# zipnn/zipnn

Measured on AMD Instinct MI355X. Metric: bf16 decompress GB/s (uncompressed bytes / s; compress GB/s beside it), higher is better.
Workload: dtype u8; 1 GPU; 4 GiB synthetic bf16 N(0,0.02) tensor per GPU, 256 KiB chunks, byte-split + huff0 (BASELINE.json configs[1]); chunks_per_gpu=16384, parallelism=chunk-sharded x1, no collectives

## Files before the change

zipnn_amd/csrc/zn_decode_chain.hpp:

```cpp
#pragma once

#include "zn_common.hpp"

#ifndef ZN_F_TLMAX
#define ZN_F_TLMAX 11u
#endif
#ifndef ZN_IN_IDX
#define ZN_IN_IDX(i) (i)
#endif
#if !defined(ZN_SIMT_EMULATOR)
#define ZN_STEP_FENCE() __builtin_amdgcn_sched_barrier(0)
#else
#define ZN_STEP_FENCE() do { } while (0)
#endif

#define ZN_E_META(cnt, nb, efields) ((nb) | ((cnt) << 8) | (efields))
#define ZN_M_NB(m) ((m) & 15u)
#define ZN_M_CNT(m) (((m) >> 8) & 7u)

__device__ __forceinline__ uint32_t zn_wave_excl_scan(uint32_t v, uint32_t lane, uint32_t* total) {
  int x = (int)v;
  x += __builtin_amdgcn_update_dpp(0, x, 0x111, 0xF, 0xF, false);
  x += __builtin_amdgcn_update_dpp(0, x, 0x112, 0xF, 0xF, false);
  x += __builtin_amdgcn_update_dpp(0, x, 0x114, 0xF, 0xF, false);
  x += __builtin_amdgcn_update_dpp(0, x, 0x118, 0xF, 0xF, false);
  x += __builtin_amdgcn_update_dpp(0, x, 0x142, 0xA, 0xF, false);
  x += __builtin_amdgcn_update_dpp(0, x, 0x143, 0xC, 0xF, false);
  *total = (uint32_t)__builtin_amdgcn_readlane(x, 63);
  (void)lane;
  return (uint32_t)x - v;
}

__device__ __forceinline__ uint64_t zn_window(const uint32_t* in, int32_t q) {
  q = q < 32 ? 32 : q;
  const int32_t j = q >> 5; const uint32_t sh = 31u - (uint32_t)(q & 31);
  const uint32_t d1 = in[ZN_IN_IDX(j)], d0 = in[ZN_IN_IDX(j - 1)];
  return (((uint64_t)d1 << 32) | d0) << sh;
}

__device__ __forceinline__ uint2 zn_trim_group(uint2 e, int32_t rem) {
  const uint32_t meta = e.y;
  const uint32_t have = ZN_M_CNT(meta);
  const uint32_t k0 = (uint32_t)(rem > 0) + (uint32_t)((int32_t)((meta >> 16) & 15u) < rem) + (uint32_t)((int32_t)((meta >> 20) & 15u) < rem) +
                      (uint32_t)((int32_t)((meta >> 24) & 15u) < rem);
  const uint32_t k = k0 < have ? k0 : have;
  const uint32_t F = ((meta >> 16) & 0xFFFu) | (ZN_M_NB(meta) << 12);
  const uint32_t nbk = k ? ((F >> (4u * k - 4u)) & 15u) : 0u;
  uint2 r;
  r.x = e.x & (k >= 4u ? 0xFFFFFFFFu : ~(0xFFFFFFFFu << (8u * k)));
  r.y = nbk | (k << 8);
  return r;
}

__device__ __forceinline__ uint2 zn_trim_group_dense(uint2 e, int32_t rem) {
  const uint32_t meta = e.y;
  const uint32_t nb = ZN_M_NB(meta), e1 = (meta >> 16) & 15u;
  const bool t0 = rem > 0, t1 = (int32_t)e1 < rem && ZN_M_CNT(meta) >= 2u;
  uint2 r;
  r.x = t1 ? e.x : (t0 ? (e.x & 0xFFu) : 0u);
  r.y = t1 ? (nb | (2u << 8)) : (t0 ? (e1 | (1u << 8)) : 0u);
  return r;
}

struct ZnChain {
  int32_t pos, stop;
  uint32_t n;
  uint32_t wpos;
};
template <int MODE>
__device__ __forceinline__ void zn_chain_apply(ZnChain& c, uint2 e, uint32_t* stage) {
  if (MODE == 2) {
    const uint64_t sp = (uint64_t)e.x << ((c.wpos & 3u) << 3);
    uint32_t* d = (uint32_t*)((uint8_t*)stage + (c.wpos & ~3u));
    if ((uint32_t)sp) atomicOr(d, (uint32_t)sp);
    if ((uint32_t)(sp >> 32)) atomicOr(d + 1, (uint32_t)(sp >> 32));
    c.wpos += ZN_M_CNT(e.y);
  }
  if (MODE == 1) c.n += ZN_M_CNT(e.y);
  c.pos -= (int32_t)ZN_M_NB(e.y);
}
template <int MODE, bool DENSE = false>
__device__ __forceinline__ void zn_fused_run(const uint2* lut, const uint32_t* in, int32_t base_bit, uint32_t TL, ZnChain& c, uint32_t* stage, int U = 0) {
  const uint32_t sh = 32u - TL;
  const int32_t mb = c.stop + (int32_t)TL - 1;
  for (int u = 0; u + 3 <= U; u += 3) {
    uint64_t w = zn_window(in, c.pos - 1 - base_bit);
    for (int s = 0; s < 3; s++) {
      const uint2 e = lut[(uint32_t)(w >> 32) >> sh];
      w <<= (e.y & 63u);
      zn_chain_apply<MODE>(c, e, stage);
    }
  }
  while (__any(c.pos > mb)) {
    uint64_t w = zn_window(in, c.pos - 1 - base_bit);
    for (int s = 0; s < 3; s++) {
      uint2 e = lut[(uint32_t)(w >> 32) >> sh];
      if (!(c.pos > mb)) { e.x = 0; e.y = 0; }
      w <<= (e.y & 63u);
      zn_chain_apply<MODE>(c, e, stage);
    }
  }
  while (__any(c.pos > c.stop)) {
    const uint64_t w = zn_window(in, c.pos - 1 - base_bit);
    uint2 e = lut[(uint32_t)(w >> 32) >> sh];
    if (!DENSE && !(c.pos > c.stop)) { e.x = 0; e.y = 0; }
    zn_chain_apply<MODE>(c, DENSE ? zn_trim_group_dense(e, c.pos - c.stop) : zn_trim_group(e, c.pos - c.stop), stage);
  }
}

#if defined(ZN_SIMT_EMULATOR)
__device__ __forceinline__ uint32_t zn_alignbyte(uint32_t hi, uint32_t lo, uint32_t sh) { return (uint32_t)(((((uint64_t)hi) << 32) | lo) >> (8u * (sh & 3u))); }
#else
__device__ __forceinline__ uint32_t zn_alignbyte(uint32_t hi, uint32_t lo, uint32_t sh) { return __builtin_amdgcn_alignbyte(hi, lo, sh); }
#endif

#define ZN_REC_LIST(X) X(0) X(1) X(2) X(3) X(4) X(5) X(6) X(7) X(8) X(9) X(10) X(11) X(12) X(13) X(14) X(15) X(16) X(17) X(18) X(19) \
                       X(20) X(21) X(22) X(23) X(24) X(25) X(26) X(27)
#define ZN_REC_MAX 28
struct ZnRec {
#define X(i) uint32_t s##i;
  ZN_REC_LIST(X)
#undef X
  uint32_t c0, c1, c2, c3, c4, c5, c6;
};
template <int I> __device__ __forceinline__ uint32_t& zn_rec_s(ZnRec& r) {
#define X(i) if constexpr (I == i) return r.s##i; else
  ZN_REC_LIST(X) return r.s0;
#undef X
}
template <int G> __device__ __forceinline__ uint32_t& zn_rec_c(ZnRec& r) {
  if constexpr (G == 0) return r.c0; else if constexpr (G == 1) return r.c1; else if constexpr (G == 2) return r.c2;
  else if constexpr (G == 3) return r.c3; else if constexpr (G == 4) return r.c4; else if constexpr (G == 5) return r.c5; else return r.c6;
}
template <int I, bool DENSE = false> __device__ __forceinline__ void zn_rec_put(ZnRec& r, uint32_t syms, uint32_t meta) {
  if constexpr (DENSE) { uint32_t& sr = zn_rec_s<I / 2>(r); if constexpr (I % 2 == 0) sr = syms; else sr = __builtin_amdgcn_perm(syms, sr, 0x05040100u); }
  else zn_rec_s<I>(r) = syms;
  constexpr uint32_t sel = (I % 4 == 0) ? 0x03020105u : (I % 4 == 1) ? 0x03020500u : (I % 4 == 2) ? 0x03050100u : 0x05020100u;
  uint32_t& c = zn_rec_c<I / 4>(r);
  c = __builtin_amdgcn_perm(meta, c, sel);
}
template <int I> __device__ __forceinline__ uint32_t zn_rec_cnt(ZnRec& r) { return (zn_rec_c<I / 4>(r) >> (8 * (I % 4))) & 7u; }
template <int I, bool DENSE> __device__ __forceinline__ uint32_t zn_rec_sym(ZnRec& r) {
  if constexpr (DENSE) return (I % 2 == 0) ? (zn_rec_s<I / 2>(r) & 0xFFFFu) : (zn_rec_s<I / 2>(r) >> 16);
  else return zn_rec_s<I>(r);
}
template <int N> struct ZnIdx { static constexpr int v = N; };
template <int I, int N, typename F> __device__ __forceinline__ void zn_static_for(F&& f) {
  if constexpr (I < N) { f(ZnIdx<I>{}); zn_static_for<I + 1, N>(f); }
}

template <int TF, int TB, int U, bool DENSE = false>
__device__ __forceinline__ bool zn_pass1(const uint2* lut, const uint32_t* in, int32_t base_bit, uint32_t TL, int32_t pos0, int32_t stop,
                                         bool own, ZnRec& rec, uint32_t& acc_out, int& nfull, int& nbnd) {
  static_assert(TF + TB <= ZN_REC_MAX, "more record slots than ZnRec has");
  const uint32_t sh = 32u - TL;
  const int32_t R = own ? pos0 - stop : -1000;
  const int32_t lim_full = R - (int32_t)TL + 1;
  const int32_t qb = pos0 - 1 - base_bit;
  uint64_t w = 0;
  uint32_t acc = 0;
  int t_end = TF; bool live = true;
  zn_static_for<0, TF>([&](auto I) {
    constexpr int t = decltype(I)::v;
    constexpr bool checked = t >= U;
    if (live) {
      bool act = true;
      if (checked) {
        act = (int32_t)(acc & 0xFFu) < lim_full;
        if (!__any(act)) { t_end = t; live = false; }
      }
      if (live) {
        if (t % 3 == 0) w = zn_window(in, qb - (int32_t)(acc & 0xFFu));
        uint2 e = lut[(uint32_t)(w >> 32) >> sh];
        if (checked && !act) { e.x = 0; e.y = 0; }
        w <<= (e.y & 63u);
        acc += e.y;
        zn_rec_put<t, DENSE>(rec, e.x, e.y);
        ZN_STEP_FENCE();
      }
    }
  });
  if (live && __any((int32_t)(acc & 0xFFu) < lim_full)) return false;
  int b_end = TB; live = true;
  zn_static_for<0, TB>([&](auto I) {
    constexpr int b = decltype(I)::v;
    if (live) {
      const int32_t rem = R - (int32_t)(acc & 0xFFu);
      if (!__any(rem > 0)) { b_end = b; live = false; }
      if (live) {
        w = zn_window(in, qb - (int32_t)(acc & 0xFFu));
        uint2 e = lut[(uint32_t)(w >> 32) >> sh];
        if (!DENSE && !(rem > 0)) { e.x = 0; e.y = 0; }
        e = DENSE ? zn_trim_group_dense(e, rem) : zn_trim_group(e, rem);
        acc += e.y;
        zn_rec_put<TF + b, DENSE>(rec, e.x, e.y);
        ZN_STEP_FENCE();
      }
    }
  });
  nfull = __builtin_amdgcn_readfirstlane(t_end); nbnd = __builtin_amdgcn_readfirstlane(b_end);
  acc_out = acc;
  return true;
}

template <int TF, int TB, bool DENSE = false, uint32_t AMASK = ~3u, typename HOOK>
__device__ __forceinline__ void zn_pass2(uint32_t* stage, uint32_t wpos, ZnRec& rec, int nfull, int nbnd, HOOK&& hook) {
  uint32_t wm1 = wpos - 1u;
  auto put = [&](uint32_t cnt, uint32_t sv) {
    const uint32_t g = ~wm1;
    uint32_t* d = (uint32_t*)((uint8_t*)stage + (int32_t)(wm1 & AMASK));
    const uint32_t lo = zn_alignbyte(sv, 0u, g), hi = zn_alignbyte(0u, sv, g);
    if (lo) atomicOr(d, lo);
    if (hi) atomicOr(d + 1, hi);
    wm1 += cnt;
    ZN_STEP_FENCE();
  };
  if constexpr (DENSE) {
    zn_static_for<0, (TF + TB + 1) / 2>([&](auto R_) {
      constexpr int r = decltype(R_)::v, a = 2 * r, b = 2 * r + 1;
      const bool va = a < TF ? a < nfull : (a - TF) < nbnd;
      const bool vb = b < TF + TB && (b < TF ? b < nfull : (b - TF) < nbnd);
      if (va || vb) {
        uint32_t ca = 0, cb = 0;
        if (va) ca = zn_rec_cnt<a>(rec);
        if constexpr (b < TF + TB) { if (vb) cb = zn_rec_cnt<b>(rec); }
        const uint32_t sr = zn_rec_s<r>(rec);
        const uint32_t sel = (ca >= 2u) ? 0x03020100u : (ca == 1u) ? 0x0c030200u : 0x0c0c0302u;
        put(ca + cb, __builtin_amdgcn_perm(sr, sr, sel));
        if (va) hook(ZnIdx<a>{});
        if constexpr (b < TF + TB) { if (vb) hook(ZnIdx<b>{}); }
      }
    });
  } else {
    zn_static_for<0, TF>([&](auto I) { constexpr int t = decltype(I)::v; if (t < nfull) { put(zn_rec_cnt<t>(rec), zn_rec_sym<t, DENSE>(rec)); hook(I); } });
    zn_static_for<0, TB>([&](auto I) { constexpr int b = decltype(I)::v; if (b < nbnd) { put(zn_rec_cnt<TF + b>(rec), zn_rec_sym<TF + b, DENSE>(rec)); hook(ZnIdx<TF + b>{}); } });
  }
}
```

zipnn_amd/csrc/zn_decode_fused.hip:

```cpp
#include "zn_internal.hpp"
#include <atomic>
#include "zn_huf_wave.hpp"
#include "zn_decode_common.hpp"
#include "zn_decode_rest.hpp"

#define ZN_F_THREADS 256
#define ZN_F_RING_BYTES 4096u
#define ZN_F_WAVES_PER_SIMD 4
#define ZN_F_RING_DW (ZN_F_RING_BYTES / 4u)
#define ZN_F_DMAX 6
#define ZN_F_DCAP 4
#define ZN_F_DOM_MAX 154
#define ZN_F_DCONST 4
#define ZN_F_DCONST2 6
#define ZN_F_DENSE_LMIN 4
#define ZN_F_IN_DW (64 * ZN_F_DMAX + 4)
#define ZN_F_TF(D) ((D) * 4 + 1)
#define ZN_F_TLMAX 11u
#define ZN_L16(i) ((i) + (((i) >> 6) << 1))
#define ZN_F_PRIO_SYNC 1
#define ZN_F_PRIO_COUNT 2
#define ZN_F_PRIO_WRITE 3
#if !defined(ZN_SIMT_EMULATOR)
#define ZN_PRIO(v) __builtin_amdgcn_s_setprio(v)
#else
#define ZN_PRIO(v) do { } while (0)
#endif
#if !defined(ZN_SIMT_EMULATOR)
#define ZN_OPAQUE32(x) asm volatile("" : "+v"(x))
#define ZN_KEEP32(x) asm volatile("" :: "v"(x))
__device__ __forceinline__ uint32_t zn_bfi_(uint32_t mask, uint32_t a, uint32_t b) {
  uint32_t d; asm("v_bfi_b32 %0, %1, %2, %3" : "=v"(d) : "s"(mask), "v"(a), "v"(b)); return d;
}
#define ZN_BFI(mask, a, b) zn_bfi_((mask), (a), (b))
#define ZN_NO_IFCVT asm volatile("")
#define ZN_ASM_MARK(txt) asm volatile("; " txt)
#else
#define ZN_NO_IFCVT ((void)0)
#define ZN_ASM_MARK(txt) ((void)0)
#define ZN_OPAQUE32(x) ((void)0)
#define ZN_KEEP32(x) ((void)(x))
#define ZN_BFI(mask, a, b) ((((uint32_t)(a)) & (uint32_t)(mask)) | (((uint32_t)(b)) & ~(uint32_t)(mask)))
#endif
#define ZN_F_DELTA0 44
#define ZN_F_DELTA0_DENSE 88
#define ZN_F_DELTA_FAST 44
#define ZN_F_DELTA_MAX 1024
#define ZN_F_NMIS 3

#if defined(ZN_SIMT_EMULATOR) && defined(ZN_DECODE_HINTED_TU)
extern unsigned long long zn_dbg_tiles[8], zn_dbg_hint[4];
#define ZN_DBG_COUNT(i) do { if (lane == 0) zn_dbg_tiles[i]++; } while (0)
#define ZN_HINT_COUNT(i, n) do { if (lane == 0) zn_dbg_hint[i] += (n); } while (0)
#define ZN_HINT_FIXUP() do { if (hinted && !hfix) { hfix = true; ZN_HINT_COUNT(1, 1); } } while (0)
#elif defined(ZN_SIMT_EMULATOR)
unsigned long long zn_dbg_tiles[8];
extern "C" void zn_debug_tile_counters(unsigned long long* out, int reset) { for (int i = 0; i < 8; i++) { out[i] = zn_dbg_tiles[i]; if (reset) zn_dbg_tiles[i] = 0; } }
#define ZN_DBG_COUNT(i) do { if (lane == 0) zn_dbg_tiles[i]++; } while (0)
unsigned long long zn_dbg_hint[4];
extern "C" void zn_debug_hint_counters(unsigned long long* out, int reset) { for (int i = 0; i < 4; i++) { out[i] = zn_dbg_hint[i]; if (reset) zn_dbg_hint[i] = 0; } }
#define ZN_HINT_COUNT(i, n) do { if (lane == 0) zn_dbg_hint[i] += (n); } while (0)
#define ZN_HINT_FIXUP() do { if (hinted && !hfix) { hfix = true; ZN_HINT_COUNT(1, 1); } } while (0)
#else
#define ZN_DBG_COUNT(i) do { } while (0)
#define ZN_HINT_COUNT(i, n) do { } while (0)
#define ZN_HINT_FIXUP() do { } while (0)
#endif

#define ZN_IN_IDX(i) (i)

#if !defined(ZN_SIMT_EMULATOR)
typedef uint32_t zn_v4u __attribute__((ext_vector_type(4)));
#define ZN_ST128(p, a, b, c, d) __builtin_nontemporal_store((zn_v4u){(a), (b), (c), (d)}, (zn_v4u*)(p))
#else
#define ZN_ST128(p, a, b, c, d) (*(uint4*)(p) = make_uint4((a), (b), (c), (d)))
#endif

#if defined(ZN_SIMT_EMULATOR)
__device__ __forceinline__ uint32_t zn_lane_id() { return threadIdx.x & 63u; }
#else
__device__ __forceinline__ uint32_t zn_lane_id() { return __builtin_amdgcn_mbcnt_hi(~0u, __builtin_amdgcn_mbcnt_lo(~0u, 0u)); }
#endif
__device__ __forceinline__ uint32_t zn_uniform(uint32_t v) { return (uint32_t)__builtin_amdgcn_readfirstlane((int)v); }
__device__ __forceinline__ uint64_t zn_uniform64(uint64_t v) { return ((uint64_t)zn_uniform((uint32_t)(v >> 32)) << 32) | zn_uniform((uint32_t)v); }
template <typename T> __device__ __forceinline__ T* zn_uniform_ptr(T* p) { return ZN_GLOBAL_PTR(T, zn_uniform64((uint64_t)p)); }

typedef uint64_t __attribute__((aligned(1))) zn_u64u;
typedef uint32_t __attribute__((aligned(1))) zn_u32u;
#if !defined(ZN_SIMT_EMULATOR)
#define ZN_LD_RAW32(p) __builtin_nontemporal_load((const zn_u32u*)(p))
#define ZN_LD_RAW64(p) __builtin_nontemporal_load((const zn_u64u*)(p))
#define ZN_LD_STREAM32(p) __builtin_nontemporal_load((const uint32_t*)(p))
#else
#define ZN_LD_RAW32(p) (*(const zn_u32u*)(p))
#define ZN_LD_RAW64(p) (*(const zn_u64u*)(p))
#define ZN_LD_STREAM32(p) (*(const uint32_t*)(p))
#endif
#if defined(ZN_SIMT_EMULATOR)
#define ZN_ST128_4(p, a, b, c, d) (*(uint4*)(p) = make_uint4((a), (b), (c), (d)))
#else
#define ZN_ST128_4(p, a, b, c, d) ZN_ST128(p, a, b, c, d)
#endif

__device__ __forceinline__ uint64_t zn_hint_header_bytes(uint64_t pk) { return ((pk + 1u) * 4u + 63u) & ~63ull; }
__device__ __forceinline__ uint32_t zn_hint_stream_bytes(uint32_t slen, uint32_t seg, uint32_t unit) {
  uint32_t d = ((ZN_F_RING_BYTES - unit - 128u) * slen) / (256u * seg);
  d = d > ZN_F_DCAP ? ZN_F_DCAP : (d < 1u ? 1u : d);
  const uint32_t dw = (slen + 6u) >> 2, td = 64u * d;
  return 64u * ((dw + td - 1u) / td);
}

struct ZnFusedPlane { uint64_t off; uint32_t kind; uint32_t csize; };

struct __attribute__((aligned(16))) ZnFusedLds {
  uint2 lut[1u << ZN_F_TLMAX];
  uint32_t ring[4][ZN_F_RING_DW];
  uint32_t in[4][ZN_F_IN_DW];
  uint8_t symlist[4][256];
  uint32_t rank_start[4][14], sym_start[4][14];
  ZnFusedPlane plane[4][4];
  ZnWaveStats st[4];
  uint32_t what[4];
};

#include "zn_decode_chain.hpp"

template <int NT = ZN_F_THREADS, typename LDS>
__device__ __forceinline__ void zn_fused_fill_luts(LDS& L, uint32_t tid, uint32_t TL, uint32_t j, uint32_t lmin = 1) {
  constexpr int KE = (int)((1u << ZN_F_TLMAX) / (uint32_t)NT);
  uint16_t* lut16 = (uint16_t*)&L.ring[0][0];
  {
    const ZnRankTab rt = zn_load_ranks(L.rank_start[j], L.sym_start[j]);
    for (uint32_t u = tid; u < (1u << TL); u += (uint32_t)NT) lut16[ZN_L16(u)] = (uint16_t)zn_lut_entry(u, TL, L.symlist[j], rt, L.rank_start[j], L.sym_start[j]);
  }
  __syncthreads();
  {
    const uint32_t mask = (1u << TL) - 1u;
    uint32_t pos[KE], cnt[KE], syms[KE], ef[KE];
    for (int k = 0; k < KE; k++) { pos[k] = 0; cnt[k] = 0; syms[k] = 0; ef[k] = 0; }
    const int rounds = (int)zn_uniform(lmin ? (TL / lmin > 4u ? 4u : TL / lmin) : 4u);
    for (int step = 0; step < 4; step++) {
      if (step >= rounds) break;
      for (int k = 0; k < KE; k++) {
        const uint32_t u = tid + (uint32_t)k * (uint32_t)NT;
        if (u <= mask && cnt[k] == (uint32_t)step) {
          const uint32_t e = lut16[ZN_L16((u << pos[k]) & mask)]; const uint32_t len = e >> 8;
          if (pos[k] + len <= TL) {
            if (step > 0) ef[k] |= pos[k] << (16 + 4 * (step - 1));
            syms[k] |= (e & 0xFFu) << (8 * step);
            pos[k] += len; cnt[k]++;
          }
        }
      }
    }
    for (int k = 0; k < KE; k++) {
      const uint32_t u = tid + (uint32_t)k * (uint32_t)NT;
      for (uint32_t i = 1; i <= 3u; i++) if (i >= cnt[k]) ef[k] |= pos[k] << (16u + 4u * (i - 1u));
      if (u <= mask) L.lut[u] = make_uint2(syms[k], ZN_E_META(cnt[k], pos[k], ef[k]));
    }
  }
}

template <int P, int H, int DC, bool X = false, int HM = 0>
__device__ __forceinline__ bool zn_fused_wave(const ZnGeom& g, const uint8_t* __restrict__ body, const uint8_t* body_end,
                                              uint8_t* outq_, const uint8_t* xq_, const ZnFusedPlane (&pl_)[P], const uint8_t* const (&rawq_)[P],
                                              const uint2* lut, uint32_t* ring, uint32_t* in, uint32_t lane_, uint32_t seg_,
                                              uint32_t TL_, uint32_t Du, const uint8_t* stream_, uint32_t slen_, bool ragged ZN_PT_PARAM,
                                              uint8_t* hq_ = nullptr, uint32_t hcap_ = 0) {
  uint32_t lane = lane_;
  uint8_t* const outq = zn_uniform_ptr(outq_); const uint8_t* const xq = zn_uniform_ptr(xq_);
  const uint8_t* const stream = zn_uniform_ptr(stream_);
  const uint32_t seg = zn_uniform(seg_), TL = zn_uniform(TL_), slen = zn_uniform(slen_);
  ZnFusedPlane pl[P]; const uint8_t* rawq[P];
  for (int p = 0; p < P; p++) {
    pl[p].off = zn_uniform64(pl_[p].off); pl[p].kind = zn_uniform(pl_[p].kind); pl[p].csize = zn_uniform(pl_[p].csize);
    rawq[p] = zn_uniform_ptr(rawq_[p]);
  }
  constexpr int EPL = (P == 1) ? 16 : 8;
  constexpr int EW = EPL / 4;
  constexpr uint32_t UNIT = 64u * EPL;
  uint8_t* const hq = HM ? zn_uniform_ptr(hq_) : nullptr; const uint32_t hcap = HM ? zn_uniform(hcap_) : 0u;
  const bool hinted = (HM == 1) && hq != nullptr;
  uint32_t ht = 0, hb_nx = 0;
#define ZN_F_RB4 2
#define ZN_F_SPLIT4 1
  constexpr bool SPLIT = (P == 4) && (ZN_F_SPLIT4 != 0);
#define ZN_F_RB2 3
  constexpr int RB = (P == 2) ? (int)ZN_F_RB2 : (P == 4) ? ZN_F_RB4 : (int)(ZN_F_RING_BYTES / 1024u);
  constexpr int TF = DC ? ZN_F_TF(DC) : 0, TB = 3;
  constexpr bool DENSE = (ZN_F_DCONST2 != 0) && (DC == ZN_F_DCONST2);
  constexpr int UF = DC ? (32 * DC - 31) / 11 : 0;
  ZN_PT_SHARED;

  uint32_t pre[RB][P][EW];
  uint32_t lane_v = lane;
  auto fetch_row_to = [&](uint32_t (&pre)[RB][P][EW], uint32_t first_row_sym, int r) {
    if constexpr (HM == 2) return;
    for (int p = 0; p < P; p++) if (p != H && pl[p].kind == ZN_KIND_RAW) {
      const uint8_t* au = rawq[p] + (first_row_sym + (uint32_t)r * UNIT);
      if constexpr (SPLIT) {
        const uint8_t* a = au + 4u * lane_v;
        pre[r][p][0] = ZN_LD_RAW32(a); pre[r][p][1 % EW] = ZN_LD_RAW32(a + UNIT / 2u);
      } else {
        const uint8_t* a = au + (uint32_t)EPL * lane_v;
        for (int k = 0; k < EW / 2; k++) { const uint64_t t = ZN_LD_RAW64(a + 8 * k); pre[r][p][2 * k] = (uint32_t)t; pre[r][p][2 * k + 1] = (uint32_t)(t >> 32); }
      }
    }
  };
  auto fetch_row = [&](uint32_t first_row_sym, int r) { fetch_row_to(pre, first_row_sym, r); };
  auto fetch_rows = [&](uint32_t first_row_sym, int nrows) {
    for (int r = 0; r < RB; r++) if (r < nrows) fetch_row_to(pre, first_row_sym, r);
  };
  auto emit_rows_from = [&](uint32_t (&pre)[RB][P][EW], bool full_wait, uint32_t first_row_sym, int nrows, uint32_t stage_row0, auto&& after_wait) {
    if (full_wait) __builtin_amdgcn_s_waitcnt(0x0F70);
    ZN_PT(10);
    after_wait();
    constexpr int XW = X ? (P == 4 ? 8 : 4) : 1, XG = 2;
    uint32_t xd[2][XG][XW];
    auto load_delta = [&](int grp) {
      for (int i = 0; i < XG; i++) {
        const int r = grp * XG + i;
        for (int k = 0; k < XW; k++) xd[grp & 1][i][k] = 0;
        if (xq && r < RB && r < nrows) {
          const uint8_t* a = SPLIT ? xq + (uint64_t)(first_row_sym + (uint32_t)r * UNIT) * P + 16u * lane
                                   : xq + (uint64_t)(first_row_sym + (uint32_t)r * UNIT + (uint32_t)EPL * lane) * P;
          for (int k = 0; k < XW / 4; k++) { const uint4 t = *(const uint4*)(a + (SPLIT ? (UNIT / 2u) * P : 16u) * k); xd[grp & 1][i][4 * k] = t.x; xd[grp & 1][i][4 * k + 1] = t.y; xd[grp & 1][i][4 * k + 2] = t.z; xd[grp & 1][i][4 * k + 3] = t.w; }
        }
      }
    };
    if (X) load_delta(0);
    for (int r = 0; r < RB; r++) if (r < nrows) {
      for (int p = 0; p < P; p++) {
        if (p == H) {
          if constexpr (SPLIT) { const uint32_t i = ((stage_row0 + (uint32_t)r) * UNIT >> 2) + lane; for (int k = 0; k < EW; k++) { pre[r][p][k] = ring[i + (UNIT / 8u) * k]; ring[i + (UNIT / 8u) * k] = 0; } }
          else { const uint32_t i = ((stage_row0 + (uint32_t)r) * UNIT + (uint32_t)EPL * lane) >> 2; for (int k = 0; k < EW; k++) { pre[r][p][k] = ring[i + k]; ring[i + k] = 0; } }
        }
        else if (pl[p].kind == ZN_KIND_RLE) { ZN_NO_IFCVT; for (int k = 0; k < EW; k++) pre[r][p][k] = ((uint32_t)pl[p].off & 0xFFu) * 0x01010101u; }
      }
    }
    if (P >= 2 && g.rot) {
      for (int r = 0; r < RB; r++) if (r < nrows)
        for (int k = 0; k < EW; k++) {
          const uint32_t hi = pre[r][P - 1][k], lo = pre[r][(P >= 2) ? P - 2 : 0][k];
          pre[r][P - 1][k] = ZN_BFI(0x80808080u, lo, hi >> 1);
          pre[r][(P >= 2) ? P - 2 : 0][k] = ZN_BFI(0x7F7F7F7Fu, lo, hi << 7);
        }
    }
    if constexpr (HM != 2)
    for (int r = 0; r < RB; r++) if (r < nrows) {
      if (X && r % XG == 0 && r + XG < RB) load_delta(r / XG + 1);
      const uint32_t* xr_ = xd[(r / XG) & 1][r % XG];
      uint8_t* o = (outq + (uint64_t)(first_row_sym + (uint32_t)r * UNIT) * P) + (SPLIT ? 16u : (uint32_t)EPL * (uint32_t)P) * lane_v;
      if (P == 1) {
        if (X) ZN_ST128(o, pre[r][0][0] ^ xr_[0], pre[r][0][1 % EW] ^ xr_[1 % XW], pre[r][0][2 % EW] ^ xr_[2 % XW], pre[r][0][3 % EW] ^ xr_[3 % XW]);
        else ZN_ST128(o, pre[r][0][0], pre[r][0][1 % EW], pre[r][0][2 % EW], pre[r][0][3 % EW]);
      } else if (P == 2) {
        uint32_t x[4];
        x[0] = __builtin_amdgcn_perm(pre[r][1 % P][0], pre[r][0][0], 0x05010400u); x[1] = __builtin_amdgcn_perm(pre[r][1 % P][0], pre[r][0][0], 0x07030602u);
        x[2] = __builtin_amdgcn_perm(pre[r][1 % P][1 % EW], pre[r][0][1 % EW], 0x05010400u); x[3] = __builtin_amdgcn_perm(pre[r][1 % P][1 % EW], pre[r][0][1 % EW], 0x07030602u);
        if (X) for (int k = 0; k < 4; k++) x[k] ^= xr_[k % XW];
        ZN_ST128(o, x[0], x[1], x[2], x[3]);
      } else {
        for (int half = 0; half < 2; half++) {
          const int k = half % EW;
          const uint32_t ab_lo = __builtin_amdgcn_perm(pre[r][1 % P][k], pre[r][0][k], 0x05010400u), ab_hi = __builtin_amdgcn_perm(pre[r][1 % P][k], pre[r][0][k], 0x07030602u);
          const uint32_t cd_lo = __builtin_amdgcn_perm(pre[r][3 % P][k], pre[r][2 % P][k], 0x05010400u), cd_hi = __builtin_amdgcn_perm(pre[r][3 % P][k], pre[r][2 % P][k], 0x07030602u);
          uint32_t x[4];
          x[0] = __builtin_amdgcn_perm(cd_lo, ab_lo, 0x05040100u); x[1] = __builtin_amdgcn_perm(cd_lo, ab_lo, 0x07060302u);
          x[2] = __builtin_amdgcn_perm(cd_hi, ab_hi, 0x05040100u); x[3] = __builtin_amdgcn_perm(cd_hi, ab_hi, 0x07060302u);
          if (X) for (int k = 0; k < 4; k++) x[k] ^= xr_[(4 * half + k) % XW];
          if constexpr (SPLIT) ZN_ST128_4(o + (UNIT / 2u) * P * half, x[0], x[1], x[2], x[3]);
          else *(uint4*)(o + 16 * half) = make_uint4(x[0], x[1], x[2], x[3]);
        }
      }
    }
  };
  auto emit_rows = [&](uint32_t first_row_sym, int nrows, uint32_t stage_row0, auto&& after_wait) { emit_rows_from(pre, true, first_row_sym, nrows, stage_row0, after_wait); };

  uint32_t JF = 0;
  if (H < 0) {
    if constexpr (HM == 2) return true;
    while (JF < seg) {
      const uint32_t left = (seg - JF) / UNIT; const int nr = left < (uint32_t)RB ? (int)left : RB;
      fetch_rows(JF, nr); emit_rows(JF, nr, 0, [] {}); JF += (uint32_t)nr * UNIT;
    }
    ZN_PT(3);
    return true;
  }

  for (uint32_t i = lane; i < ZN_F_RING_DW; i += 64u) ring[i] = 0;
  __builtin_amdgcn_wave_barrier();

  uint32_t J = 0;
  const uint8_t last = stream[slen - 1];
  if (last == 0) return false;
  const uint32_t mis = (uint32_t)((uint64_t)stream & 3u);
  const uint32_t* gdw = (const uint32_t*)(stream - mis);
  const int32_t b0 = (int32_t)(8u * mis);
  int32_t carry = __builtin_amdgcn_readfirstlane(b0 + (int32_t)(8u * (slen - 1u)) + (int32_t)zn_hb32(last));
  int32_t hi_dw = (carry + 31) >> 5;
  const int32_t Di = DC ? DC : (int32_t)Du, TD = 64 * Di;
  int32_t delta = (DENSE ? ZN_F_DELTA0_DENSE : ZN_F_DELTA0) < 32 * Di ? (DENSE ? ZN_F_DELTA0_DENSE : ZN_F_DELTA0) : 32 * Di;
  int nmis = 0;

  uint32_t nx[ZN_F_DMAX], nx_last = 0;
  const int32_t top_dw = hi_dw - 1;
  const bool top_guard = ((const uint8_t*)(gdw + hi_dw) > body_end);
  auto fetch_tile = [&](int32_t lo_dw_, int32_t hi_dw_) {
    const uint32_t* pu = gdw + (lo_dw_ - 1);
    if (lo_dw_ >= 0 && !(top_guard && hi_dw_ - 1 == top_dw)) {
      for (int i = 0; i < ZN_F_DMAX; i++) nx[i] = (i < Di) ? ZN_LD_STREAM32(pu + (lane_v + 64u * (uint32_t)i)) : 0u;
      nx_last = gdw[__builtin_amdgcn_readfirstlane(hi_dw_) - 1];
    } else {
      auto dword_at = [&](int32_t li) -> uint32_t {
        const int32_t gi = lo_dw_ - 1 + li;
        uint32_t x = 0;
        if (li <= TD && gi >= -1 && gi < hi_dw_) {
          if (top_guard && gi == top_dw) { const uint8_t* pa = (const uint8_t*)(gdw + gi); for (int b = 0; b < 4; b++) if (pa + b < body_end) x |= (uint32_t)pa[b] << (8 * b); }
          else x = gdw[gi];
        }
        return x;
      };
      for (int i = 0; i < ZN_F_DMAX; i++) nx[i] = (i < Di) ? dword_at((int32_t)lane + 64 * i) : 0u;
      nx_last = (lane == 0) ? dword_at(TD) : 0u;
    }
  };
  auto stage_tile = [&]() {
    __builtin_amdgcn_wave_barrier();
    for (int i = 0; i < ZN_F_DMAX; i++) if (i < Di) in[ZN_IN_IDX((int32_t)lane + 64 * i)] = nx[i];
    if (lane == 0) in[ZN_IN_IDX(TD)] = nx_last;
    __builtin_amdgcn_wave_barrier();
  };
  auto fetch_hint = [&](uint32_t t) {
    if constexpr (HM == 1) { hb_nx = 0; if (hinted && 64u * t + 64u <= hcap) hb_nx = hq[64u * t + lane_v]; }
  };
  fetch_hint(0);
  fetch_tile(hi_dw - TD, hi_dw);
  stage_tile();

  auto sync_run = [&](int32_t base_bit, int32_t hi_k, bool active, bool regular_tile) -> int32_t {
    ZnChain c;
    c.pos = (lane > 0 && active) ? hi_k + delta : hi_k; c.stop = hi_k; c.n = 0; c.wpos = 0;
    if (delta <= ZN_F_DELTA_FAST) {
      const uint32_t sh = 32u - TL;
      const int G = delta <= 22 ? 2 : delta <= 33 ? 3 : 4;
      uint64_t w = zn_window(in, c.pos - 1 - base_bit);
      auto group = [&]() { uint2 e = lut[(uint32_t)(w >> 32) >> sh]; if (!(c.pos > c.stop + (int32_t)TL - 1)) { e.x = 0; e.y = 0; } w <<= (e.y & 63u); c.pos -= (int32_t)ZN_M_NB(e.y); };
      group(); group();
      if (G >= 3) { ZN_NO_IFCVT; group(); w = zn_window(in, c.pos - 1 - base_bit); }
      if (G >= 4) { ZN_NO_IFCVT; group(); }
      { uint2 e = lut[(uint32_t)(w >> 32) >> sh]; if (!(c.pos > c.stop)) { e.x = 0; e.y = 0; } c.pos -= (int32_t)ZN_M_NB(zn_trim_group(e, c.pos - c.stop).y); }
      while (__any(c.pos > c.stop)) {
        w = zn_window(in, c.pos - 1 - base_bit);
        uint2 e = lut[(uint32_t)(w >> 32) >> sh]; if (!(c.pos > c.stop)) { e.x = 0; e.y = 0; }
        c.pos -= (int32_t)ZN_M_NB(zn_trim_group(e, c.pos - c.stop).y);
      }
    } else {
      zn_fused_run<0, DENSE>(lut, in, base_bit, TL, c, nullptr, regular_tile ? (delta - 21) / 11 : 0);
    }
    return (lane > 0) ? c.pos : carry;
  };
  auto note_mismatch = [&]() { if (++nmis >= ZN_F_NMIS) { nmis = 0; delta = (delta < 22) ? 22 : (delta < ZN_F_DELTA_FAST) ? delta + 11 : 2 * delta; if (delta > 32 * Di) delta = 32 * Di; if (delta > ZN_F_DELTA_MAX) delta = ZN_F_DELTA_MAX; } };
  auto keep_remainder = [&](uint32_t total_rows) {
    const uint32_t i = (total_rows * UNIT + (uint32_t)EPL * lane) >> 2;
    uint32_t t[EW];
    for (int k = 0; k < EW; k++) { t[k] = ring[i + k]; ring[i + k] = 0; }
    __builtin_amdgcn_wave_barrier();
    for (int k = 0; k < EW; k++) ring[((uint32_t)EPL * lane >> 2) + k] = t[k];
    __builtin_amdgcn_wave_barrier();
  };

  bool ok = true;
  while (32 * hi_dw > b0) {
    if (DC) ZN_ASM_MARK("ZN_HOT_TILE_BEGIN");
    lane = zn_lane_id();
    lane_v = lane; ZN_OPAQUE32(lane_v);
    hi_dw = __builtin_amdgcn_readfirstlane(hi_dw); carry = __builtin_amdgcn_readfirstlane(carry);
    delta = __builtin_amdgcn_readfirstlane(delta); nmis = __builtin_amdgcn_readfirstlane(nmis);
    J = zn_uniform(J); JF = zn_uniform(JF);
    const int32_t lo_dw = hi_dw - TD;
    const uint32_t hb = hb_nx, ht_cur = ht; ht++;
    if (32 * lo_dw > b0) { fetch_hint(ht); fetch_tile(lo_dw - TD, lo_dw); }
    ZN_PT(4);
    const int32_t base_bit = 32 * (lo_dw - 1);
    const int32_t hi_k = 32 * (hi_dw - (int32_t)lane * Di), lo_k = hi_k - 32 * Di;
    const int32_t stop = lo_k > b0 ? lo_k : b0;
    const bool active = hi_k > b0;
    const bool regular = (32 * lo_dw >= b0);
    ZN_PT_COUNT(18, 1);
    ZN_DBG_COUNT(0);
    if (HM == 1) { if (hinted) ZN_HINT_COUNT(0, 1); else ZN_HINT_COUNT(2, 1); }
    bool hfix = false; (void)hfix;
    auto hint_start = [&]() -> int32_t {
      const uint32_t g4 = hb & 15u; const int32_t gg = (int32_t)(g4 > 10u ? 10u : g4);
      const int32_t sh_ = hi_k - gg;
      return (lane > 0) ? (active ? (sh_ > stop ? sh_ : stop) : hi_k) : carry;
    };
    auto hint_store = [&](int32_t s_final) {
      if constexpr (HM == 2) {
        if (hq && 64u * ht_cur + 64u <= hcap) { hq[64u * ht_cur + lane_v] = (uint8_t)((lane > 0 && active) ? ((uint32_t)(hi_k - s_final) & 15u) : 0u); ZN_HINT_COUNT(3, 64); }
      }
    };

    bool done = false;
    if (TF > 0) {
      ZN_PRIO(ZN_F_PRIO_SYNC);
      if (DC) ZN_ASM_MARK("ZN_MARK sync");
      int32_t s;
      if (HM == 1 && hinted) s = hint_start(); else s = sync_run(base_bit, hi_k, active, regular);
      ZN_PRIO(ZN_F_PRIO_COUNT);
      ZN_PT(5);
      if (DC) ZN_ASM_MARK("ZN_MARK pass1");
      ZnRec rec;
      int nfull = 0, nbnd = 0;
      uint32_t acc = 0, n = 0; int32_t e = s;
      bool took = true, chained = false;
      for (int it = 0; it < 4; it++) {
        if (regular) took = zn_pass1<TF, TB, UF, DENSE>(lut, in, base_bit, TL, s, stop, true, rec, acc, nfull, nbnd);
        else took = zn_pass1<TF, TB, 0, DENSE>(lut, in, base_bit, TL, s, stop, active, rec, acc, nfull, nbnd);
        if (!took) break;
        e = s - (int32_t)(acc & 0xFFu); n = (acc >> 8) & 0xFFu;
        const int32_t e_prev = __shfl_up(e, 1u);
        const bool mism = active && lane > 0 && e_prev != s;
        if (it == 0) ZN_PT(6); else ZN_PT(7);
        if (__builtin_expect(!__any(mism), 1)) { chained = true; break; }
        ZN_PT_COUNT(16, 1);
        ZN_PT_COUNT(17, __popcll(__ballot(mism)));
        ZN_DBG_COUNT(2);
        ZN_HINT_FIXUP();
        if (it == 0 && !(HM == 1 && hinted)) note_mismatch();
        if (mism) s = e_prev;
      }
      if (DC) ZN_ASM_MARK("ZN_MARK scan");
      if (took && chained) {
        if (!active) n = 0;
        uint32_t N = 0;
        const uint32_t o_k = zn_wave_excl_scan(n, lane, &N);
        J = zn_uniform(J); JF = zn_uniform(JF);
        const uint32_t base = J - JF;
        if (J + N <= seg && base + N <= ZN_F_RING_BYTES - 4u) {
          const uint32_t nact = (uint32_t)__popcll(__ballot(active));
          carry = __builtin_amdgcn_readlane(e, (int)(nact ? nact - 1u : 0u)); hi_dw = lo_dw;
          hint_store(s);
          int rows = (int)zn_uniform((base + N) / UNIT);
          const uint32_t total_rows = (uint32_t)rows;
          const int first = rows < RB ? rows : RB;
          constexpr int RH = (RB >= 4) ? RB / 2 : RB;
          for (int r = 0; r < RH; r++) if (r < first) fetch_row(JF, r);
          ZN_PT(8);
          ZN_PRIO(ZN_F_PRIO_WRITE);
          if (DC) ZN_ASM_MARK("ZN_MARK pass2");
          const int nf = __builtin_amdgcn_readfirstlane(nfull), nb_ = __builtin_amdgcn_readfirstlane(nbnd);
          bool late_rows = (RH < RB);
          zn_pass2<TF, TB, DENSE>(ring, base + o_k, rec, nf, nb_, [&](auto I) {
            if constexpr (RH < RB && decltype(I)::v == TF / 2 - 1) { for (int r = RH; r < RB; r++) if (r < first) fetch_row(JF, r); late_rows = false; }
          });
          if (late_rows) for (int r = RH; r < RB; r++) if (r < first) fetch_row(JF, r);
          __builtin_amdgcn_wave_barrier();
          ZN_PRIO(0);
          ZN_PT(9);
          if (DC) ZN_ASM_MARK("ZN_MARK flush");
          J += N;
          emit_rows(JF, first, 0, [&] {
            if (32 * hi_dw > b0) stage_tile();
          });
          uint32_t srow = (uint32_t)first;
          JF += (uint32_t)first * UNIT; rows -= first;
          while (rows > 0) { const int nr = rows < RB ? rows : RB; fetch_rows(JF, nr); emit_rows(JF, nr, srow, [] {}); JF += (uint32_t)nr * UNIT; srow += (uint32_t)nr; rows -= nr; }
          if (total_rows > 0 && J > JF) keep_remainder(total_rows);
          ZN_PT_COUNT(20, 1);
          if (DC) ZN_ASM_MARK("ZN_MARK fastend");
          done = true;
        }
      }
    }

    if (!done) {
      ZN_NO_IFCVT;
      ZN_PT_COUNT(22, 1);
      ZN_DBG_COUNT(1);
      ZN_PRIO(ZN_F_PRIO_SYNC);
      int32_t s;
      if (HM == 1 && hinted) s = hint_start(); else s = sync_run(base_bit, hi_k, active, regular);
      ZN_PRIO(ZN_F_PRIO_COUNT);
      ZnChain A; A.wpos = 0;
      const int U_blk = regular ? (int)zn_uniform((uint32_t)((32 * Di - 31) / 11)) : 0;
      int32_t e = s; uint32_t n = 0; bool need = active, chained = false;
      for (int it = 0; it < 66; it++) {
        A.pos = need ? s : stop; A.stop = stop; A.n = 0;
        zn_fused_run<1>(lut, in, base_bit, TL, A, nullptr, U_blk);
        if (need) { e = A.pos; n = A.n; }
        const int32_t e_prev = __shfl_up(e, 1u);
        const bool mism = active && lane > 0 && e_prev != s;
        if (!__any(mism)) { chained = true; break; }
        ZN_HINT_FIXUP();
        if (it == 0 && !(HM == 1 && hinted)) note_mismatch();
        need = mism;
        if (mism) s = e_prev;
      }
      if (!active) n = 0;
      uint32_t N = 0;
      const uint32_t o_k = zn_wave_excl_scan(n, lane, &N);
      const uint32_t nact = (uint32_t)__popcll(__ballot(active));
      const int32_t e_last = __builtin_amdgcn_readlane(e, (int)(nact ? nact - 1u : 0u));
      if (!chained || J + N > seg) { ok = false; break; }
      carry = e_last; hi_dw = lo_dw;
      hint_store(s);
      uint32_t lane_lo = 0, wdone = 0;
      do {
        const uint32_t base = J - JF;
        const bool fits = o_k + n <= wdone + (ZN_F_RING_BYTES - 4u - base);
        const uint32_t lane_hi = (uint32_t)__popcll(__ballot(fits));
        if (lane_hi <= lane_lo) { ok = false; break; }
        if (lane_hi < 64u) ZN_DBG_COUNT(3);
        const uint32_t wend = (lane_hi >= 64u) ? N : (uint32_t)__shfl((int)o_k, (int)(lane_hi & 63u));
        const uint32_t nsub = wend - wdone;
        int rows = (int)((base + nsub) / UNIT);
        const int first = rows < RB ? rows : RB;
        fetch_rows(JF, first);
        ZN_PRIO(ZN_F_PRIO_WRITE);
        const bool mine = active && lane >= lane_lo && lane < lane_hi;
        A.pos = mine ? s : stop; A.stop = stop; A.wpos = mine ? base + o_k - wdone : 0u;
        zn_fused_run<2>(lut, in, base_bit, TL, A, ring, (lane_lo == 0u && lane_hi >= 64u) ? U_blk : 0);
        __builtin_amdgcn_wave_barrier();
        ZN_PRIO(0);
        J += nsub; wdone = wend; lane_lo = lane_hi;
        const uint32_t total_rows = (uint32_t)rows;
        uint32_t srow = 0;
        emit_rows(JF, first, srow, [&] {
          if (lane_hi >= 64u && 32 * hi_dw > b0) stage_tile();
        });
        JF += (uint32_t)first * UNIT; srow += (uint32_t)first; rows -= first;
        while (rows > 0) { const int nr = rows < RB ? rows : RB; fetch_rows(JF, nr); emit_rows(JF, nr, srow, [] {}); JF += (uint32_t)nr * UNIT; srow += (uint32_t)nr; rows -= nr; }
        if (total_rows > 0 && J > JF) keep_remainder(total_rows);
        ZN_PT_COUNT(20, 1);
      } while (lane_lo < 64u);
      if (!ok) break;
    }
    ZN_PT(3);
    if (DC) ZN_ASM_MARK("ZN_HOT_TILE_END");
  }
  ZN_PRIO(0);
  if (ragged && ok && carry == b0 && J == seg && JF < seg) {
    emit_rows(JF, 1, 0, [] {}); JF += UNIT;
  }
  return ok && carry == b0 && J == seg && JF >= seg;
}

template <int P>
__device__ __forceinline__ void zn_tail_merge_wg(ZnFusedLds& L, const ZnSeg& one_c, const ZnSeg* __restrict__ segs, uint32_t nseg, uint32_t m, uint32_t merge_per,
                                                 uint32_t* __restrict__ tailsync, ZnPlaneDesc* __restrict__ descs_rest, uint32_t* __restrict__ status,
                                                 uint8_t* __restrict__ tail_done, uint8_t* __restrict__ tail_scratch) {
  const uint32_t tt = m / merge_per, jm = m % merge_per;
  const ZnSeg S = zn_find_seg<3>(one_c, segs, nseg, (uint64_t)tt * (uint32_t)P);
  const uint32_t tid = threadIdx.x, lane = tid & 63u, wave = (uint32_t)__builtin_amdgcn_readfirstlane((int)(tid >> 6));
  const uint64_t c = S.g.K - 1u;
  __shared__ uint32_t ok_s, serial_s;
  if (tid == 0) { ok_s = zn_flag_wait(tailsync + 2u * tt, 4u * (uint32_t)P) ? 1u : 0u; serial_s = 0; ZN_FLAG_ACQUIRE(); }
  __syncthreads();
  if (!ok_s) { if (tid == 0) atomicOr(status, ZN_DEV_SYNC_TIMEOUT); return; }
  static_assert(4u * sizeof(ZnPlanesLds) <= sizeof(ZnFusedLds), "four generic plane decoders fit over the fused kernel's LDS");
  if (wave < (uint32_t)P) zn_decode_plane_item(reinterpret_cast<ZnPlanesLds*>(&L)[wave], one_c, segs, nseg, S.desc0 + (uint64_t)wave * S.g.K + c, descs_rest, status, tail_done, lane, true, &serial_s);
  __syncthreads();
  if (tid == 0) ZN_FLAG_ACQUIRE();
  __syncthreads();
  uint32_t sub = jm, nsub = merge_per;
  if (serial_s) {
    if (jm != 0u) return;
    if (wave < (uint32_t)P) zn_decode_plane_item(reinterpret_cast<ZnPlanesLds*>(&L)[wave], one_c, segs, nseg, S.desc0 + (uint64_t)wave * S.g.K + c, descs_rest, status, tail_done, lane);
    __threadfence(); __syncthreads();
    sub = 0; nsub = 1;
  }
  zn_merge_chunk_item<P>(one_c, segs, nseg, S.chunk0 + c, sub, descs_rest, tail_scratch, nsub);
}

#if defined(ZN_DECODE_HINTED_TU)
#define ZN_TU_LOCAL static
#else
#define ZN_TU_LOCAL
#endif
ZN_TU_LOCAL __device__ void zn_decode_tail_wg(ZnFusedLds& L_, const ZnSeg& one, const ZnSeg* __restrict__ segs, uint32_t nseg, uint32_t bt,
                                  uint8_t* __restrict__ scratch, uint8_t* __restrict__ tail_done, uint32_t* __restrict__ status, uint32_t* tail0_out);
#include "zn_decode_wide.hpp"

ZN_TU_LOCAL __device__ void zn_decode_tail_wg(ZnFusedLds& L_, const ZnSeg& one, const ZnSeg* __restrict__ segs, uint32_t nseg, uint32_t bt,
                                  uint8_t* __restrict__ scratch, uint8_t* __restrict__ tail_done, uint32_t* __restrict__ status, uint32_t* tail0_out) {
  ZnFusedLds& L = *ZN_LDS_PTR(ZnFusedLds, &L_);
  const uint32_t b = bt >> 2, sq = zn_uniform(bt & 3u);
  const ZnSeg S = zn_find_seg<3>(one, segs, nseg, b);
  *tail0_out = S.tail0;
  const ZnGeom g = S.g;
  const uint8_t* __restrict__ body = ZN_GLOBAL_PTR(const uint8_t, S.body); const uint64_t body_len = S.body_len;
  const uint8_t* body_end = body + body_len;
  const uint32_t tid = threadIdx.x, lane = tid & 63u, wave = (uint32_t)__builtin_amdgcn_readfirstlane((int)(tid >> 6));
  const uint32_t p = b - S.tail0;
  const uint64_t c = g.K - 1u;
  ZN_PT_DECL;
  const ZnPcMeta m = zn_pc_meta(g, S.kb, S.c_lo, body, body_len, p, c);
  if (!(m.ok && m.type == 1u && m.csize > 1u && m.csize < m.plen && m.plen >= ZN_TAIL_WG_MIN_PLANE && m.plen <= 4u * ZN_TAIL_SEGPAD)) return;
  const uint8_t* src = body + m.off;
  if (wave == 0) {
    uint8_t* tmp = (uint8_t*)&L.ring[0][0];
    const ZnWaveStats st = zn_wave_read_stats(src, m.csize, body_end, lane, tmp, L.symlist[0], L.rank_start[0], L.sym_start[0], tmp + 512);
    if (lane == 0) L.st[0] = st;
  }
  __syncthreads();
  const ZnWaveStats st = L.st[0];
// ... 488 lines not shown
```

Baseline: 2910 GB/s.

## Store running byte counts in pass1 records and unguard the regular sync run-in

Pass1 now records the running accumulator instead of per-step counts, so pass2 computes each write address as base plus the prior running count rather than a serial add chain. The LDS base pointer is also folded into the write offset so the per-put address arithmetic shrinks. For regular tiles at the default delta, the sync run-in drops its per-group guard and selects, decoding four groups unconditionally. This relies on the tile invariant that all lanes have room for four 11-bit groups. Emulator-only counters and asserts are added to check that assumption.

```diff
diff --git a/zipnn_amd/csrc/zn_decode_chain.hpp b/zipnn_amd/csrc/zn_decode_chain.hpp
--- a/zipnn_amd/csrc/zn_decode_chain.hpp
+++ b/zipnn_amd/csrc/zn_decode_chain.hpp
@@ -12,6 +12,14 @@
 #define ZN_STEP_FENCE() __builtin_amdgcn_sched_barrier(0)
 #else
 #define ZN_STEP_FENCE() do { } while (0)
+#endif
+
+#if defined(ZN_SIMT_EMULATOR) || !defined(__HIP_DEVICE_COMPILE__)
+typedef uintptr_t zn_lds_addr;
+#define ZN_LDS_ADDR(p) ((zn_lds_addr)(p))
+#else
+typedef uint32_t zn_lds_addr;
+#define ZN_LDS_ADDR(p) ((zn_lds_addr)(unsigned long long)(p))
 #endif
 
 #define ZN_E_META(cnt, nb, efields) ((nb) | ((cnt) << 8) | (efields))
@@ -114,6 +122,10 @@
 __device__ __forceinline__ uint32_t zn_alignbyte(uint32_t hi, uint32_t lo, uint32_t sh) { return __builtin_amdgcn_alignbyte(hi, lo, sh); }
 #endif
 
+#ifndef ZN_DIET_PASS2
+#define ZN_DIET_PASS2 1
+#endif
+
 #define ZN_REC_LIST(X) X(0) X(1) X(2) X(3) X(4) X(5) X(6) X(7) X(8) X(9) X(10) X(11) X(12) X(13) X(14) X(15) X(16) X(17) X(18) X(19) \
                        X(20) X(21) X(22) X(23) X(24) X(25) X(26) X(27)
 #define ZN_REC_MAX 28
@@ -132,12 +144,18 @@
   if constexpr (G == 0) return r.c0; else if constexpr (G == 1) return r.c1; else if constexpr (G == 2) return r.c2;
   else if constexpr (G == 3) return r.c3; else if constexpr (G == 4) return r.c4; else if constexpr (G == 5) return r.c5; else return r.c6;
 }
+template <int I> __device__ __forceinline__ void zn_rec_put_cnt(ZnRec& r, uint32_t meta) {
+  constexpr uint32_t sel = (I % 4 == 0) ? 0x03020105u : (I % 4 == 1) ? 0x03020500u : (I % 4 == 2) ? 0x03050100u : 0x05020100u;
+  uint32_t& c = zn_rec_c<I / 4>(r);
+  c = __builtin_amdgcn_perm(meta, c, sel);
+}
 template <int I, bool DENSE = false> __device__ __forceinline__ void zn_rec_put(ZnRec& r, uint32_t syms, uint32_t meta) {
   if constexpr (DENSE) { uint32_t& sr = zn_rec_s<I / 2>(r); if constexpr (I % 2 == 0) sr = syms; else sr = __builtin_amdgcn_perm(syms, sr, 0x05040100u); }
   else zn_rec_s<I>(r) = syms;
-  constexpr uint32_t sel = (I % 4 == 0) ? 0x03020105u : (I % 4 == 1) ? 0x03020500u : (I % 4 == 2) ? 0x03050100u : 0x05020100u;
-  uint32_t& c = zn_rec_c<I / 4>(r);
-  c = __builtin_amdgcn_perm(meta, c, sel);
+  zn_rec_put_cnt<I>(r, meta);
+}
+template <int I> __device__ __forceinline__ uint32_t zn_rec_before(ZnRec& r) {
+  if constexpr (I == 0) return 0u; else return (zn_rec_c<(I - 1) / 4>(r) >> (8 * ((I - 1) % 4))) & 0xFFu;
 }
 template <int I> __device__ __forceinline__ uint32_t zn_rec_cnt(ZnRec& r) { return (zn_rec_c<I / 4>(r) >> (8 * (I % 4))) & 7u; }
 template <int I, bool DENSE> __device__ __forceinline__ uint32_t zn_rec_sym(ZnRec& r) {
@@ -149,7 +167,7 @@
   if constexpr (I < N) { f(ZnIdx<I>{}); zn_static_for<I + 1, N>(f); }
 }
 
-template <int TF, int TB, int U, bool DENSE = false>
+template <int TF, int TB, int U, bool DENSE = false, bool RUNCNT = false>
 __device__ __forceinline__ bool zn_pass1(const uint2* lut, const uint32_t* in, int32_t base_bit, uint32_t TL, int32_t pos0, int32_t stop,
                                          bool own, ZnRec& rec, uint32_t& acc_out, int& nfull, int& nbnd) {
   static_assert(TF + TB <= ZN_REC_MAX, "more record slots than ZnRec has");
@@ -175,12 +193,13 @@
         if (checked && !act) { e.x = 0; e.y = 0; }
         w <<= (e.y & 63u);
         acc += e.y;
-        zn_rec_put<t, DENSE>(rec, e.x, e.y);
+        zn_rec_put<t, DENSE>(rec, e.x, RUNCNT ? acc : e.y);
         ZN_STEP_FENCE();
       }
     }
   });
   if (live && __any((int32_t)(acc & 0xFFu) < lim_full)) return false;
+  if constexpr (RUNCNT) zn_rec_put_cnt<TF - 1>(rec, acc);
   int b_end = TB; live = true;
   zn_static_for<0, TB>([&](auto I) {
     constexpr int b = decltype(I)::v;
@@ -193,7 +212,7 @@
         if (!DENSE && !(rem > 0)) { e.x = 0; e.y = 0; }
         e = DENSE ? zn_trim_group_dense(e, rem) : zn_trim_group(e, rem);
         acc += e.y;
-        zn_rec_put<TF + b, DENSE>(rec, e.x, e.y);
+        zn_rec_put<TF + b, DENSE>(rec, e.x, RUNCNT ? acc : e.y);
         ZN_STEP_FENCE();
       }
     }
@@ -203,18 +222,25 @@
   return true;
 }
 
-template <int TF, int TB, bool DENSE = false, uint32_t AMASK = ~3u, typename HOOK>
+template <int TF, int TB, bool DENSE = false, uint32_t AMASK = ~3u, bool RUNCNT = false, typename HOOK>
 __device__ __forceinline__ void zn_pass2(uint32_t* stage, uint32_t wpos, ZnRec& rec, int nfull, int nbnd, HOOK&& hook) {
-  uint32_t wm1 = wpos - 1u;
+  static_assert(!(RUNCNT && DENSE), "the dense records keep the steps' own counts");
+  constexpr bool FOLD = (ZN_DIET_PASS2 != 0) && AMASK == ~3u, RUN = RUNCNT;
+  const zn_lds_addr wm0 = (zn_lds_addr)(intptr_t)(int32_t)(wpos - 1u) + (FOLD ? ZN_LDS_ADDR(stage) : (zn_lds_addr)0);
+  zn_lds_addr wm1 = wm0;
   auto put = [&](uint32_t cnt, uint32_t sv) {
-    const uint32_t g = ~wm1;
-    uint32_t* d = (uint32_t*)((uint8_t*)stage + (int32_t)(wm1 & AMASK));
+    const uint32_t g = ~(uint32_t)wm1;
+    uint32_t* d;
+    if constexpr (FOLD) d = ZN_LDS_PTR(uint32_t, wm1 & ~(zn_lds_addr)3);
+    else d = (uint32_t*)((uint8_t*)stage + (int32_t)((uint32_t)wm1 & AMASK));
     const uint32_t lo = zn_alignbyte(sv, 0u, g), hi = zn_alignbyte(0u, sv, g);
     if (lo) atomicOr(d, lo);
     if (hi) atomicOr(d + 1, hi);
-    wm1 += cnt;
+    if constexpr (!RUN) wm1 += cnt;
     ZN_STEP_FENCE();
   };
+  auto put_at = [&](auto I, uint32_t sv) { wm1 = wm0 + zn_rec_before<decltype(I)::v>(rec); put(0u, sv); };
+  (void)put_at;
   if constexpr (DENSE) {
     zn_static_for<0, (TF + TB + 1) / 2>([&](auto R_) {
       constexpr int r = decltype(R_)::v, a = 2 * r, b = 2 * r + 1;
@@ -232,7 +258,7 @@
       }
     });
   } else {
-    zn_static_for<0, TF>([&](auto I) { constexpr int t = decltype(I)::v; if (t < nfull) { put(zn_rec_cnt<t>(rec), zn_rec_sym<t, DENSE>(rec)); hook(I); } });
-    zn_static_for<0, TB>([&](auto I) { constexpr int b = decltype(I)::v; if (b < nbnd) { put(zn_rec_cnt<TF + b>(rec), zn_rec_sym<TF + b, DENSE>(rec)); hook(ZnIdx<TF + b>{}); } });
-  }
-}
+    zn_static_for<0, TF>([&](auto I) { constexpr int t = decltype(I)::v; if (t < nfull) { if constexpr (RUN) put_at(I, zn_rec_sym<t, DENSE>(rec)); else put(zn_rec_cnt<t>(rec), zn_rec_sym<t, DENSE>(rec)); hook(I); } });
+    zn_static_for<0, TB>([&](auto I) { constexpr int b = decltype(I)::v; if (b < nbnd) { if constexpr (RUN) put_at(ZnIdx<TF + b>{}, zn_rec_sym<TF + b, DENSE>(rec)); else put(zn_rec_cnt<TF + b>(rec), zn_rec_sym<TF + b, DENSE>(rec)); hook(ZnIdx<TF + b>{}); } });
+  }
+}
diff --git a/zipnn_amd/csrc/zn_decode_fused.hip b/zipnn_amd/csrc/zn_decode_fused.hip
--- a/zipnn_amd/csrc/zn_decode_fused.hip
+++ b/zipnn_amd/csrc/zn_decode_fused.hip
@@ -1,5 +1,8 @@
 #include "zn_internal.hpp"
 #include <atomic>
+#if defined(ZN_SIMT_EMULATOR)
+#include <cassert>
+#endif
 #include "zn_huf_wave.hpp"
 #include "zn_decode_common.hpp"
 #include "zn_decode_rest.hpp"
@@ -46,23 +49,34 @@
 #define ZN_F_DELTA0_DENSE 88
 #define ZN_F_DELTA_FAST 44
 #define ZN_F_DELTA_MAX 1024
+#ifndef ZN_DIET_RUNIN
+#define ZN_DIET_RUNIN 1
+#endif
 #define ZN_F_NMIS 3
 
 #if defined(ZN_SIMT_EMULATOR) && defined(ZN_DECODE_HINTED_TU)
-extern unsigned long long zn_dbg_tiles[8], zn_dbg_hint[4];
+extern unsigned long long zn_dbg_tiles[8], zn_dbg_hint[4], zn_dbg_runin[12];
+extern int zn_dbg_delta0;
 #define ZN_DBG_COUNT(i) do { if (lane == 0) zn_dbg_tiles[i]++; } while (0)
+#define ZN_RUNIN_COUNT(i) do { if (lane == 0) zn_dbg_runin[i]++; } while (0)
 #define ZN_HINT_COUNT(i, n) do { if (lane == 0) zn_dbg_hint[i] += (n); } while (0)
 #define ZN_HINT_FIXUP() do { if (hinted && !hfix) { hfix = true; ZN_HINT_COUNT(1, 1); } } while (0)
 #elif defined(ZN_SIMT_EMULATOR)
 unsigned long long zn_dbg_tiles[8];
 extern "C" void zn_debug_tile_counters(unsigned long long* out, int reset) { for (int i = 0; i < 8; i++) { out[i] = zn_dbg_tiles[i]; if (reset) zn_dbg_tiles[i] = 0; } }
 #define ZN_DBG_COUNT(i) do { if (lane == 0) zn_dbg_tiles[i]++; } while (0)
+unsigned long long zn_dbg_runin[12];
+int zn_dbg_delta0 = 0;
+extern "C" void zn_debug_set_runin(int bits) { zn_dbg_delta0 = bits; }
+extern "C" void zn_debug_runin_counters(unsigned long long* out, int reset) { for (int i = 0; i < 12; i++) { out[i] = zn_dbg_runin[i]; if (reset) zn_dbg_runin[i] = 0; } }
+#define ZN_RUNIN_COUNT(i) do { if (lane == 0) zn_dbg_runin[i]++; } while (0)
 unsigned long long zn_dbg_hint[4];
 extern "C" void zn_debug_hint_counters(unsigned long long* out, int reset) { for (int i = 0; i < 4; i++) { out[i] = zn_dbg_hint[i]; if (reset) zn_dbg_hint[i] = 0; } }
 #define ZN_HINT_COUNT(i, n) do { if (lane == 0) zn_dbg_hint[i] += (n); } while (0)
 #define ZN_HINT_FIXUP() do { if (hinted && !hfix) { hfix = true; ZN_HINT_COUNT(1, 1); } } while (0)
 #else
 #define ZN_DBG_COUNT(i) do { } while (0)
+#define ZN_RUNIN_COUNT(i) do { } while (0)
 #define ZN_HINT_COUNT(i, n) do { } while (0)
 #define ZN_HINT_FIXUP() do { } while (0)
 #endif
@@ -190,6 +204,7 @@
   constexpr int TF = DC ? ZN_F_TF(DC) : 0, TB = 3;
   constexpr bool DENSE = (ZN_F_DCONST2 != 0) && (DC == ZN_F_DCONST2);
   constexpr int UF = DC ? (32 * DC - 31) / 11 : 0;
+  constexpr bool RUNCNT = (ZN_DIET_PASS2 != 0) && !DENSE;
   ZN_PT_SHARED;
 
   uint32_t pre[RB][P][EW];
@@ -301,6 +316,9 @@
   int32_t hi_dw = (carry + 31) >> 5;
   const int32_t Di = DC ? DC : (int32_t)Du, TD = 64 * Di;
   int32_t delta = (DENSE ? ZN_F_DELTA0_DENSE : ZN_F_DELTA0) < 32 * Di ? (DENSE ? ZN_F_DELTA0_DENSE : ZN_F_DELTA0) : 32 * Di;
+#if defined(ZN_SIMT_EMULATOR)
+  if (!DENSE && zn_dbg_delta0 > 0 && zn_dbg_delta0 < delta) delta = zn_dbg_delta0;
+#endif
   int nmis = 0;
 
   uint32_t nx[ZN_F_DMAX], nx_last = 0;
@@ -346,9 +364,23 @@
       const int G = delta <= 22 ? 2 : delta <= 33 ? 3 : 4;
       uint64_t w = zn_window(in, c.pos - 1 - base_bit);
       auto group = [&]() { uint2 e = lut[(uint32_t)(w >> 32) >> sh]; if (!(c.pos > c.stop + (int32_t)TL - 1)) { e.x = 0; e.y = 0; } w <<= (e.y & 63u); c.pos -= (int32_t)ZN_M_NB(e.y); };
-      group(); group();
-      if (G >= 3) { ZN_NO_IFCVT; group(); w = zn_window(in, c.pos - 1 - base_bit); }
-      if (G >= 4) { ZN_NO_IFCVT; group(); }
+      if (ZN_DIET_RUNIN && regular_tile && delta == ZN_F_DELTA0) {
+        ZN_NO_IFCVT;
+        static_assert(ZN_F_DELTA0 == 44 && ZN_F_TLMAX <= 11u, "the unguarded run-in is four groups of at most 11 bits");
+        ZN_RUNIN_COUNT(0);
+        auto group_u = [&]() {
+#if defined(ZN_SIMT_EMULATOR)
+          assert(lane == 0 || (active && c.pos > c.stop + (int32_t)TL - 1));
+#endif
+          const uint2 e = lut[(uint32_t)(w >> 32) >> sh]; w <<= (e.y & 63u); c.pos -= (int32_t)ZN_M_NB(e.y);
+        };
+        group_u(); group_u(); group_u(); w = zn_window(in, c.pos - 1 - base_bit); group_u();
+      } else {
+        ZN_RUNIN_COUNT(1);
+        group(); group();
+        if (G >= 3) { ZN_NO_IFCVT; group(); w = zn_window(in, c.pos - 1 - base_bit); }
+        if (G >= 4) { ZN_NO_IFCVT; group(); }
+      }
       { uint2 e = lut[(uint32_t)(w >> 32) >> sh]; if (!(c.pos > c.stop)) { e.x = 0; e.y = 0; } c.pos -= (int32_t)ZN_M_NB(zn_trim_group(e, c.pos - c.stop).y); }
       while (__any(c.pos > c.stop)) {
         w = zn_window(in, c.pos - 1 - base_bit);
@@ -356,6 +388,7 @@
         c.pos -= (int32_t)ZN_M_NB(zn_trim_group(e, c.pos - c.stop).y);
       }
     } else {
+      ZN_RUNIN_COUNT(2);
       zn_fused_run<0, DENSE>(lut, in, base_bit, TL, c, nullptr, regular_tile ? (delta - 21) / 11 : 0);
     }
     return (lane > 0) ? c.pos : carry;
@@ -416,8 +449,8 @@
       uint32_t acc = 0, n = 0; int32_t e = s;
       bool took = true, chained = false;
       for (int it = 0; it < 4; it++) {
-        if (regular) took = zn_pass1<TF, TB, UF, DENSE>(lut, in, base_bit, TL, s, stop, true, rec, acc, nfull, nbnd);
-        else took = zn_pass1<TF, TB, 0, DENSE>(lut, in, base_bit, TL, s, stop, active, rec, acc, nfull, nbnd);
+        if (regular) took = zn_pass1<TF, TB, UF, DENSE, RUNCNT>(lut, in, base_bit, TL, s, stop, true, rec, acc, nfull, nbnd);
+        else took = zn_pass1<TF, TB, 0, DENSE, RUNCNT>(lut, in, base_bit, TL, s, stop, active, rec, acc, nfull, nbnd);
         if (!took) break;
         e = s - (int32_t)(acc & 0xFFu); n = (acc >> 8) & 0xFFu;
         const int32_t e_prev = __shfl_up(e, 1u);
@@ -438,7 +471,13 @@
         const uint32_t o_k = zn_wave_excl_scan(n, lane, &N);
         J = zn_uniform(J); JF = zn_uniform(JF);
         const uint32_t base = J - JF;
+        if (J + N <= seg && base + N > ZN_F_RING_BYTES - 4u) ZN_RUNIN_COUNT(9);
         if (J + N <= seg && base + N <= ZN_F_RING_BYTES - 4u) {
+#if defined(ZN_SIMT_EMULATOR)
+          { const uint32_t r_ = (base + N) % UNIT;
+            if (r_ == 0u) ZN_RUNIN_COUNT(4); if (r_ == UNIT - 1u) ZN_RUNIN_COUNT(5); if (r_ == 1u) ZN_RUNIN_COUNT(6);
+            if (base == 0u && N > 0u) ZN_RUNIN_COUNT(7); if (base + N > ZN_F_RING_BYTES - 8u) ZN_RUNIN_COUNT(8); }
+#endif
           const uint32_t nact = (uint32_t)__popcll(__ballot(active));
           carry = __builtin_amdgcn_readlane(e, (int)(nact ? nact - 1u : 0u)); hi_dw = lo_dw;
           hint_store(s);
@@ -452,7 +491,7 @@
           if (DC) ZN_ASM_MARK("ZN_MARK pass2");
           const int nf = __builtin_amdgcn_readfirstlane(nfull), nb_ = __builtin_amdgcn_readfirstlane(nbnd);
           bool late_rows = (RH < RB);
-          zn_pass2<TF, TB, DENSE>(ring, base + o_k, rec, nf, nb_, [&](auto I) {
+          zn_pass2<TF, TB, DENSE, ~3u, RUNCNT>(ring, base + o_k, rec, nf, nb_, [&](auto I) {
             if constexpr (RH < RB && decltype(I)::v == TF / 2 - 1) { for (int r = RH; r < RB; r++) if (r < first) fetch_row(JF, r); late_rows = false; }
           });
           if (late_rows) for (int r = RH; r < RB; r++) if (r < first) fetch_row(JF, r);
```

After: 2910 GB/s, median of 2. No clear change (+0.0%).
